# adithom/KWS

Measured on AMD Instinct MI355X. Metric: utterances/sec fwd+bwd, T=99 feat=32 hidden=128, bs=4096 at 1/2/4/8 GPUs, higher is better.
Workload: dtype f32 (split-precision MFMA: exact 3xbf16 planes, fp16 two-plane forward state product; fp32 accumulate)

## Files before the change

include/fastgrnn_hip.h:

```cpp
#ifndef FASTGRNN_HIP_H
#define FASTGRNN_HIP_H

#include <stddef.h>
#include <stdint.h>

#ifdef __cplusplus
extern "C" {
#endif

#define FASTGRNN_HIP_ABI_VERSION 1

typedef enum fastgrnn_status {
  FASTGRNN_OK = 0,
  FASTGRNN_ERR_NULL_POINTER = 1,
  FASTGRNN_ERR_BAD_SHAPE = 2,
  FASTGRNN_ERR_BAD_NONLINEARITY = 3,
  FASTGRNN_ERR_BAD_DTYPE = 4,
  FASTGRNN_ERR_WORKSPACE = 5,
  FASTGRNN_ERR_LAUNCH = 6,
  FASTGRNN_ERR_UNSUPPORTED = 7
} fastgrnn_status;

typedef enum fastgrnn_dtype {
  FASTGRNN_F32 = 0,
  FASTGRNN_F64 = 1,
  FASTGRNN_BF16_IO = 2
} fastgrnn_dtype;

typedef enum fastgrnn_nonlinearity {
  FASTGRNN_NL_SIGMOID = 0, FASTGRNN_NL_RELU = 1, FASTGRNN_NL_TANH = 2,
  FASTGRNN_NL_QUANT_TANH = 3, FASTGRNN_NL_QUANT_SIGM = 4, FASTGRNN_NL_QUANT_SIGM4 = 5
} fastgrnn_nonlinearity;

#define FASTGRNN_FLAG_FORCE_GENERIC 1u
#define FASTGRNN_FLAG_FORCE_F32_MFMA 2u
#define FASTGRNN_FLAG_SAVE_PREACT 4u
#define FASTGRNN_FLAG_FWD_4WAVE 8u
#define FASTGRNN_FLAG_BATCH_MAJOR 16u
#define FASTGRNN_FLAG_X_BFT 128u
#define FASTGRNN_FLAG_FWD_BF16X3 64u
#define FASTGRNN_FLAG_GRAD_LAST 256u
#define FASTGRNN_FLAG_HS_LAST 512u
#define FASTGRNN_FLAG_PREACT_AFFINE 1024u
#define FASTGRNN_FLAG_BN_TRAIN 2048u
#define FASTGRNN_FLAG_ZERO_EXTEND 4096u
#define FASTGRNN_FLAG_NO_INPUT_GRAD 8192u

typedef struct fastgrnn_desc {
  int32_t T, B, F, H;
  int32_t w_rank, u_rank;
  int32_t gate_nl;
  int32_t update_nl;
  int32_t dtype;
  uint32_t flags;
} fastgrnn_desc;

typedef struct fastgrnn_params {
  const void *w, *u;
  const void *w1, *w2, *u1, *u2;
  const void *bias_gate;
  const void *bias_update;
  const void *zeta, *nu;
} fastgrnn_params;

typedef struct fastgrnn_grads {
  void *d_x;
  void *d_bias_gate;
  void *d_bias_update;
  void *d_zeta;
  void *d_nu;
  void *d_h0;
  void *d_w, *d_u;
  void *d_w1, *d_w2;
  void *d_u1, *d_u2;
} fastgrnn_grads;

int fastgrnn_hip_abi_version(void);
const char *fastgrnn_hip_status_string(int status);

int fastgrnn_hip_kernel_path(const fastgrnn_desc *d, int direction);

typedef struct fastgrnn_zext_plan {
  int32_t forward, backward;
  int32_t Hp, Fp;
  int32_t dx_optional, reserved;
  size_t saved_bytes;
} fastgrnn_zext_plan;
int fastgrnn_hip_zero_extend_plan(const fastgrnn_desc *d, fastgrnn_zext_plan *out);

typedef struct fastgrnn_plan {
// ... 224 lines not shown
```

kws_amd/_lib.py:

```python
from __future__ import annotations

import ctypes as C
import os

_HERE = os.path.dirname(os.path.abspath(__file__))
LIB_PATH = os.environ.get("FASTGRNN_HIP_LIB") or os.path.join(_HERE, "csrc", "libfastgrnn_hip.so")

ABI_VERSION = 1

F32, F64, BF16_IO = 0, 1, 2
FLAG_FORCE_GENERIC = 1
FLAG_FORCE_F32_MFMA = 2
FLAG_SAVE_PREACT = 4
FLAG_FWD_4WAVE = 8
FLAG_FWD_BF16X3 = 64
FLAG_X_BFT = 128
FLAG_GRAD_LAST = 256
FLAG_HS_LAST = 512
FLAG_BATCH_MAJOR = 16
FLAG_PREACT_AFFINE = 1024
FLAG_BN_TRAIN = 2048
FLAG_ZERO_EXTEND = 4096
FLAG_NO_INPUT_GRAD = 8192

NONLINEARITY = {"sigmoid": 0, "relu": 1, "tanh": 2, "quantTanh": 3, "quantSigm": 4, "quantSigm4": 5}

EXPORTS = (
    "fastgrnn_hip_abi_version", "fastgrnn_hip_status_string", "fastgrnn_hip_kernel_path",
    "fastgrnn_hip_forward_workspace_bytes", "fastgrnn_hip_backward_workspace_bytes",
    "fastgrnn_hip_forward_unroll", "fastgrnn_hip_backward_unroll",
    "fastgrnn_hip_forward", "fastgrnn_hip_backward",
    "fastgrnn_hip_head_workspace_bytes", "fastgrnn_hip_head_xent", "fastgrnn_hip_debug_poison_cu_state",
    "fastgrnn_hip_frame_gemm", "fastgrnn_hip_forward_unroll_affine",
    "fastgrnn_hip_bn_train_supported", "fastgrnn_hip_bn_train_forward_workspace_bytes",
    "fastgrnn_hip_bn_train_backward_workspace_bytes", "fastgrnn_hip_bn_train_forward", "fastgrnn_hip_bn_train_backward",
    "fastgrnn_hip_zero_extend_plan", "fastgrnn_hip_plan",
    "fastgrnn_hip_windows_supported", "fastgrnn_hip_forward_windows_workspace_bytes", "fastgrnn_hip_forward_windows",
    "fastgrnn_hip_train_windows_supported", "fastgrnn_hip_train_windows_forward_workspace_bytes",
    "fastgrnn_hip_train_windows_backward_workspace_bytes", "fastgrnn_hip_forward_windows_train",
    "fastgrnn_hip_backward_windows",
    "fastgrnn_hip_head_predict_workspace_bytes", "fastgrnn_hip_head_predict", "fastgrnn_hip_vote_windows",
    "fastgrnn_hip_train_update", "fastgrnn_hip_optim_update",
    "fastgrnn_hip_mfcc_tables_bytes", "fastgrnn_hip_mfcc_init_tables", "fastgrnn_hip_mfcc_workspace_bytes",
    "fastgrnn_hip_mfcc", "fastgrnn_hip_mfcc_augment", "fastgrnn_hip_augment_draw", "fastgrnn_hip_train_schedule",
)


class Desc(C.Structure):
    _fields_ = [("T", C.c_int32), ("B", C.c_int32), ("F", C.c_int32), ("H", C.c_int32),
                ("w_rank", C.c_int32), ("u_rank", C.c_int32),
                ("gate_nl", C.c_int32), ("update_nl", C.c_int32),
                ("dtype", C.c_int32), ("flags", C.c_uint32)]


class Params(C.Structure):
    _fields_ = [(n, C.c_void_p) for n in
                ("w", "u", "w1", "w2", "u1", "u2", "bias_gate", "bias_update", "zeta", "nu")]


class Grads(C.Structure):
    _fields_ = [(n, C.c_void_p) for n in
                ("d_x", "d_bias_gate", "d_bias_update", "d_zeta", "d_nu", "d_h0",
                 "d_w", "d_u", "d_w1", "d_w2", "d_u1", "d_u2")]


class BnLayer(C.Structure):
    _fields_ = [("gamma", C.c_void_p), ("beta", C.c_void_p), ("running_mean", C.c_void_p),
                ("running_var", C.c_void_p), ("num_batches_tracked", C.c_void_p),
                ("eps", C.c_double), ("momentum", C.c_double)]


class BnParams(C.Structure):
    _fields_ = [("w", BnLayer), ("u", BnLayer), ("gate", BnLayer), ("update", BnLayer)]


class BnGrads(C.Structure):
# ... 208 lines not shown
```

kws_amd/csrc/kernels_split.hip:

```cpp
#include "split_common.h"

namespace fastgrnn {
namespace {

template <int GATE, int AUX, bool RAGGED>
__global__ __launch_bounds__(256) ONE_WAVE_PER_SIMD void fwd_scan_split(
    int Tn, int B, int rsT, int rsB, const float* __restrict__ x, const float* __restrict__ h0,
    const float* __restrict__ w, const float* __restrict__ u,
    const float* __restrict__ bz, const float* __restrict__ bh,
    const float* __restrict__ zeta, const float* __restrict__ nu,
    float* __restrict__ hs, float* __restrict__ zs, float* __restrict__ cs) {
  constexpr int H = 128, F = 32, MT = 2, KS = H / 32;
  __shared__ u32x4 hl[2][3][KS * 4 * 16];

  const int tid = threadIdx.x;
  const int wv = __builtin_amdgcn_readfirstlane(tid >> 6);
  const int l = tid & 63, i = l & 15, g = l >> 4;
  const int b = blockIdx.x * 16 + i;
  const bool valid = !RAGGED || b < B;
  const int bc = valid ? b : B - 1;
  const int n0 = wv * 32 + g * 8;
  const int myfrag = (wv * 4 + g) * 16 + i;

  Frag3 Uf[MT][KS], Wf[MT];
// ... 364 lines not shown
      st4(zs + o, zq); st4(cs + o, cq);
    }
    aux_prev = a;
    publish_h(cur ^ 1);
    SPLIT_STAMP(3)
    lds_barrier();
    SPLIT_STAMP(4)
  }
#ifdef FASTGRNN_DIAG_STAMPS
  if (blockIdx.x == 7 && l == 0) { for (int k2 = 0; k2 < 8; ++k2) g_sdiag[wv][k2] = dsum[k2]; }
#endif
  store_step(Tn - 1, aux_prev);
  };
  if constexpr (F16H) {
    if (use_h16) scan(std::true_type{}); else scan(std::false_type{});
  } else {
    scan(std::false_type{});
  }
}



constexpr int SLAB = (128 * 128 + 128 * 32 + 2 * 128 + 2 + 63) & ~63;

constexpr int ROW_H = 288;
constexpr int ROW_X = 96;
constexpr int PLANE_H = 16 * ROW_H;
constexpr int PLANE_X = 16 * ROW_X;
constexpr int IMG = 2 * 3 * PLANE_H + 3 * PLANE_X;

constexpr int OFF_DP = 0, OFF_HP = 3 * PLANE_H, OFF_XP = 6 * PLANE_H;

template <bool WITH_DX>
struct BwdW8Lds {
  unsigned char img[4][IMG];
  f32x4 DX[2][8][64];
  float bias[2][128];
  float red[16];
};
template <>
struct BwdW8Lds<false> {
  unsigned char img[4][IMG];
  float bias[2][128];
  float red[16];
};

constexpr bool bwd_w8_built(int gate, bool preact, bool bf, bool nox, bool uq, bool nodx) {
  const bool ref_gate = gate <= FASTGRNN_NL_TANH;
  if (nox) return !uq && !nodx && (!bf || (ref_gate && preact));
  if (uq) return preact && !bf;
  if (bf) return preact;
  return true;
}
template <int GATE, bool PREACT, bool RAGGED, bool BF = false, bool NOX = false, bool UQ = false, bool NODX = false>
__global__ __launch_bounds__(512) void bwd_scan_split_w8(
    int Tn, int B, int rsT, int rsB, int mode, const float* __restrict__ ghs, const float* __restrict__ x,
    const float* __restrict__ hs, const float* __restrict__ aux0, const float* __restrict__ aux1,
    const float* __restrict__ h0, const float* __restrict__ w, const float* __restrict__ u,
    const float* __restrict__ bz, const float* __restrict__ bh,
    const float* __restrict__ zeta, const float* __restrict__ nu,
    float* __restrict__ d_x, float* __restrict__ d_h0, float* __restrict__ part) {
  constexpr int H = 128, F = 32, KS = 4, NFT = NOX ? 0 : 2, NC = NOX ? 4 : 5;
  constexpr bool STATIC_TURNS = !NOX, SELECT_AT_USE = !NOX;
  static_assert(!(NOX && NODX), "NOX scans leave d_x to a GEMM of its own");
  __shared__ BwdW8Lds<!NODX> S;
#ifdef FASTGRNN_DIAG_STAMPS
  unsigned long long dsum[8] = {0, 0, 0, 0, 0, 0, 0, 0}, dlast = 0;
  asm volatile("s_memtime %0\n\ts_waitcnt lgkmcnt(0)" : "=s"(dlast)::"memory");
#endif

  const bool xbft = (mode & 1) != 0, g_last = (mode & 2) != 0;
  const int tid = threadIdx.x;
  const int wv = __builtin_amdgcn_readfirstlane(tid >> 6);
  const int l = tid & 63, i = l & 15, g = l >> 4;
  const int b = blockIdx.x * 16 + i;
  const bool valid = !RAGGED || b < B;
  const int bc = valid ? b : B - 1;
  const int n0 = wv * 16 + g * 4;
  const float sz = fsigmoid(zeta[0]), sn = fsigmoid(nu[0]);
  if (Tn & 1) {
    for (int idx = tid; idx < IMG / 4; idx += 512) reinterpret_cast<unsigned*>(&S.img[Tn & 3][0])[idx] = 0u;
  }
  if (PREACT && tid < 256) S.bias[tid >> 7][tid & 127] = (tid < 128 ? bz : bh)[tid & 127];

  Frag3 UTf[KS];
#pragma unroll
  for (int s2 = 0; s2 < KS; ++s2) {
    f32x4 lo, hi;
#pragma unroll
    for (int j = 0; j < 4; ++j) {
      lo[j] = u[(size_t)(32 * s2 + 8 * g + j) * H + wv * 16 + i];
      hi[j] = u[(size_t)(32 * s2 + 8 * g + 4 + j) * H + wv * 16 + i];
    }
    UTf[s2] = split3(lo, hi);
  }
  const int xf2 = wv & 1, xks = wv >> 1;
  Frag3 WTf;
  if (!NOX && !NODX) {
    f32x4 lo, hi;
#pragma unroll
    for (int j = 0; j < 4; ++j) {
      lo[j] = w[(size_t)(32 * xks + 8 * g + j) * F + xf2 * 16 + i];
      hi[j] = w[(size_t)(32 * xks + 8 * g + 4 + j) * F + xf2 * 16 + i];
    }
    WTf = split3(lo, hi);
  }
  f32x4 sbz = f32x4{0.f, 0.f, 0.f, 0.f}, sbh = sbz, dh = sbz;
  float pz = 0.f, pn = 0.f, pz_c = 0.f, pn_c = 0.f;
  auto role_body = [&](auto role_tag) __attribute__((always_inline)) {
  const int rp = wv & 3;
  constexpr int ch = decltype(role_tag)::value;
  f32x4 acc[2][NC];
#pragma unroll
  for (int a = 0; a < 2; ++a)
#pragma unroll
    for (int c = 0; c < NC; ++c) acc[a][c] = f32x4{0.f, 0.f, 0.f, 0.f};

  const unsigned lds_img = (unsigned)(size_t)&S.img[0][0];
  const unsigned my_row_h = (unsigned)(i * ROW_H + n0 * 2);
  const int xu = tid >> 5, xf = tid & 31;
  const unsigned my_x = (unsigned)(xu * ROW_X + xf * 2);
  const int xbb = blockIdx.x * 16 + xu;
  const int xbc = (!RAGGED || xbb < B) ? xbb : B - 1;
  const int q = (l & 15) >> 2, pp = l & 3;
  const unsigned trA_off = OFF_DP + (8 * (g & 1) + q) * ROW_H + (rp * 32 + 4 * pp) * 2;
  const unsigned trH_off = OFF_HP + (8 * (g & 1) + q) * ROW_H + (4 * pp) * 2;
  const unsigned trX_off = OFF_XP + (8 * (g & 1) + q) * ROW_X + (4 * pp) * 2;

  auto fragments_landed = [&]() __attribute__((always_inline)) { __builtin_amdgcn_sched_barrier(0); };
  struct EwOps { f32x4 g, a0, a1, h; float xv; uint2 graw, hraw; unsigned short xraw; };
  constexpr unsigned ESZ = BF ? 2u : 4u;
  const unsigned lane_e = (unsigned)bc * (unsigned)rsB * H + n0;
  const unsigned lane_bh = (unsigned)bc * H + n0;
  const unsigned dp_step = (NOX && valid) ? (unsigned)rsT * H * 4u : 0u;
  const unsigned dp_off = !NOX ? 0u : (valid ? ((unsigned)b * (unsigned)rsB * H + n0) * 4u
                                             : (((unsigned)Tn * (unsigned)B + i) * H + n0) * 4u);
  const unsigned lane_x = NOX ? 0u : (xbft ? ((unsigned)xbc * F + xf) * (unsigned)Tn : (unsigned)xbc * (unsigned)rsB * F + xf);
  auto ldg4 = [](const void* base, unsigned byte_off) __attribute__((always_inline)) {
    return *reinterpret_cast<const f32x4*>(reinterpret_cast<const char*>(base) + byte_off);
  };
  auto ldg2 = [](const void* base, unsigned byte_off) __attribute__((always_inline)) {
    return *reinterpret_cast<const uint2*>(reinterpret_cast<const char*>(base) + byte_off);
  };
  auto load_ew = [&](int t, EwOps& e) __attribute__((always_inline)) {
    const size_t step_h = (size_t)t * rsT * H;
    e.a0 = ldg4(aux0 + step_h, lane_e * 4u);
    if (!PREACT) e.a1 = ldg4(aux1 + step_h, lane_e * 4u);
    const char* gbase = g_last ? reinterpret_cast<const char*>(ghs) : reinterpret_cast<const char*>(ghs) + step_h * ESZ;
    const unsigned goff = (g_last ? lane_bh : lane_e) * ESZ;
    const char* hbase = (t == 0) ? reinterpret_cast<const char*>(hs)
                                 : reinterpret_cast<const char*>(hs) + (step_h - (size_t)rsT * H) * ESZ;
    const char* xbase = xbft ? reinterpret_cast<const char*>(x) + (size_t)t * ESZ
                             : reinterpret_cast<const char*>(x) + (size_t)t * rsT * F * ESZ;
    const bool g_zero = g_last && t != Tn - 1;
    if (BF) {
      e.graw = ldg2(gbase, goff);
      if constexpr (!SELECT_AT_USE) {
        e.graw = g_zero ? uint2{0u, 0u} : e.graw;
        if (RAGGED && !valid) e.graw = uint2{0u, 0u};
      }
      e.hraw = ldg2(hbase, lane_e * ESZ);
      if (t == 0) e.h = ldg4(h0, lane_bh * 4u);
      if (!NOX) e.xraw = *reinterpret_cast<const unsigned short*>(xbase + lane_x * ESZ);
    } else {
      e.g = ldg4(gbase, goff);
      if constexpr (!SELECT_AT_USE) {
        e.g = g_zero ? f32x4{0.f, 0.f, 0.f, 0.f} : e.g;
        if (RAGGED && !valid) e.g = f32x4{0.f, 0.f, 0.f, 0.f};
      }
      e.h = (t == 0) ? ldg4(h0, lane_bh * 4u) : ldg4(hbase, lane_e * 4u);
      if (!NOX) e.xv = *reinterpret_cast<const float*>(xbase + lane_x * 4u);
    }
  };
  auto unpack4 = [](const uint2 v) __attribute__((always_inline)) {
    return f32x4{__builtin_bit_cast(float, v.x << 16), __builtin_bit_cast(float, v.x & 0xFFFF0000u),
                 __builtin_bit_cast(float, v.y << 16), __builtin_bit_cast(float, v.y & 0xFFFF0000u)};
  };
  auto unpack_ew = [&](int t, EwOps& e) __attribute__((always_inline)) {
    if (BF) {
      e.g = unpack4(e.graw);
      if (t != 0) e.h = unpack4(e.hraw);
      if (!NOX) e.xv = bf16_to_f32(e.xraw);
    }
    if constexpr (SELECT_AT_USE) {
      const bool g_zero = g_last && t != Tn - 1;
      e.g = g_zero ? f32x4{0.f, 0.f, 0.f, 0.f} : e.g;
      if (RAGGED && !valid) e.g = f32x4{0.f, 0.f, 0.f, 0.f};
    }
  };
  struct EwPre { f32x4 kc, kz, z, c; };
  auto ew_pre = [&](const EwOps& e, EwPre& f) __attribute__((always_inline)) {
    f32x4 bzq = f32x4{0.f, 0.f, 0.f, 0.f}, bhq = bzq;
    if (PREACT) {
      bzq = *reinterpret_cast<const f32x4*>(&S.bias[0][n0]);
      bhq = *reinterpret_cast<const f32x4*>(&S.bias[1][n0]);
    }
#pragma unroll
    for (int r = 0; r < 4; ++r) {
      float z, c;
      if (PREACT) {
        z = gate_act<GATE>(e.a0[r] + bzq[r]);
        c = UQ ? fminf(fmaxf(e.a0[r] + bhq[r], -1.0f), 1.0f) : ftanh(e.a0[r] + bhq[r]);
      } else {
        z = e.a0[r]; c = e.a1[r];
      }
      const float dc = UQ ? ((c < 1.0f && c > -1.0f) ? 1.0f : 0.0f) : 1.0f - c * c;
      f.kc[r] = (sz * (1.0f - z) + sn) * dc;
      f.kz[r] = (e.h[r] - sz * c) * gate_dact<GATE>(z);
      f.z[r] = z; f.c[r] = c;
    }
  };
  auto put4 = [&](unsigned char* base, int plane_stride, unsigned off, const f32x4 v) __attribute__((always_inline)) {
    uint2 q0, q1, q2;
    split_quad(v, q0, q1, q2);
    *reinterpret_cast<uint2*>(base + off) = q0;
    *reinterpret_cast<uint2*>(base + plane_stride + off) = q1;
    *reinterpret_cast<uint2*>(base + 2 * plane_stride + off) = q2;
  };
  auto ew_post = [&](int t, const EwOps& e, const EwPre& f, const f32x4 ggv) __attribute__((always_inline)) {
    f32x4 dpv;
    float sn4 = 0.f, sz4 = 0.f;
#pragma unroll
    for (int r = 0; r < 4; ++r) {
      const float gg = ggv[r];
      const float dcp = f.kc[r] * gg, dzp = f.kz[r] * gg;
      sbz[r] += dzp; sbh[r] += dcp;
      const float cg = f.c[r] * gg;
      if constexpr (NOX) { sn4 += cg; sz4 += cg - f.z[r] * cg; }
      else { pn += cg; pz += cg - f.z[r] * cg; }
      dpv[r] = dzp + dcp;
      dh[r] = f.z[r] * gg;
    }
    if constexpr (NOX) { kahan_add(pn, pn_c, sn4); kahan_add(pz, pz_c, sz4); }
    unsigned char* im = &S.img[t & 3][0];
    put4(im + OFF_DP, PLANE_H, my_row_h, dpv);
    put4(im + OFF_HP, PLANE_H, my_row_h, e.h);
    if (NOX) {
      *reinterpret_cast<f32x4*>(reinterpret_cast<char*>(d_x) + (size_t)t * dp_step + dp_off) = dpv;
    } else {
      unsigned short s0, s1, s2;
      split_one(e.xv, s0, s1, s2);
      *reinterpret_cast<unsigned short*>(im + OFF_XP + my_x) = s0;
      *reinterpret_cast<unsigned short*>(im + OFF_XP + PLANE_X + my_x) = s1;
      *reinterpret_cast<unsigned short*>(im + OFF_XP + 2 * PLANE_X + my_x) = s2;
    }
  };
  auto finish_dx = [&](int t) __attribute__((always_inline)) {
    if constexpr (!NOX && !NODX) {
      if (wv < NFT) {
        const f32x4 sacc = (S.DX[t & 1][wv][l] + S.DX[t & 1][wv + 2][l]) + (S.DX[t & 1][wv + 4][l] + S.DX[t & 1][wv + 6][l]);
        if (xbft) {
          if (valid) {
#pragma unroll
            for (int r = 0; r < 4; ++r) {
              const size_t o = ((size_t)b * F + wv * 16 + 4 * g + r) * Tn + t;
              if (BF) reinterpret_cast<unsigned short*>(d_x)[o] = (unsigned short)f32_to_bf16_rne(sacc[r]);
              else d_x[o] = sacc[r];
            }
          }
        } else {
          char* xo = reinterpret_cast<char*>(d_x) + (size_t)t * rsT * F * ESZ;
          const unsigned lo = ((unsigned)b * (unsigned)rsB * F + wv * 16 + 4 * g) * ESZ;
          if (valid) { if (BF) st4_bf16(xo + lo, sacc); else *reinterpret_cast<f32x4*>(xo + lo) = sacc; }
        }
      }
    }
  };
  auto weight_grads = [&](auto pure_tag, int sU) __attribute__((always_inline)) {
    constexpr bool PURE3 = decltype(pure_tag)::value;
    const unsigned im = lds_img + (unsigned)(((g < 2) ? sU : sU - 1) & 3) * IMG;
    const unsigned trA = im + trA_off, trH = im + trH_off, trX = im + trX_off;
    Frag3 Af[2];
#pragma unroll
    for (int a2 = 0; a2 < 2; ++a2)
#pragma unroll
      for (int pl = 0; pl < 3; ++pl) Af[a2].p[pl] = tr_frag(trA + pl * PLANE_H + a2 * 32, ROW_H);
    auto load_b = [&](int c, Frag3& bf) __attribute__((always_inline)) {
      const int ct = NC * ch + c;
#pragma unroll
      for (int pl = 0; pl < 3; ++pl)
        bf.p[pl] = (ct < NFT) ? tr_frag(trX + pl * PLANE_X + ct * 32, ROW_X)
                              : tr_frag(trH + pl * PLANE_H + (ct - NFT) * 32, ROW_H);
    };
    auto batch = [&](auto c0_tag, auto n_tag) __attribute__((always_inline)) {
      constexpr int C0 = decltype(c0_tag)::value, NB = decltype(n_tag)::value;
      Frag3 Bf[NB];
#pragma unroll
      for (int c = 0; c < NB; ++c) load_b(C0 + c, Bf[c]);
      fragments_landed();
      if constexpr (PURE3) {
#pragma unroll
        for (int c = 0; c < NB; ++c)
#pragma unroll
          for (int a2 = 0; a2 < 2; ++a2) {
            f32x4 v = mfma_bf16(Af[a2].p[2], Bf[c].p[0], acc[a2][C0 + c]);
            v = mfma_bf16(Af[a2].p[1], Bf[c].p[0], v);
            acc[a2][C0 + c] = mfma_bf16(Af[a2].p[0], Bf[c].p[0], v);
          }
      } else {
#pragma unroll
        for (int c = 0; c < NB; ++c)
#pragma unroll
          for (int a2 = 0; a2 < 2; ++a2) acc[a2][C0 + c] = mfma6(Af[a2], Bf[c], acc[a2][C0 + c]);
      }
      __builtin_amdgcn_sched_barrier(0);
      float touch = 0.f;
#pragma unroll
      for (int c = 0; c < NB; ++c) touch += acc[0][C0 + c][0] + acc[1][C0 + c][0];
      completion_read(touch);
      __builtin_amdgcn_sched_barrier(0);
    };
    constexpr bool ONE_TILE_BATCHES = PREACT && GATE == FASTGRNN_NL_TANH && !NOX;
    if constexpr (ONE_TILE_BATCHES) {
      static_for<NC>([&](auto c_tag) __attribute__((always_inline)) { batch(c_tag, std::integral_constant<int, 1>{}); });
    } else {
      batch(std::integral_constant<int, 0>{}, std::integral_constant<int, 2>{});
      batch(std::integral_constant<int, 2>{}, std::integral_constant<int, 2>{});
      if constexpr (NC == 5) batch(std::integral_constant<int, 4>{}, std::integral_constant<int, 1>{});
    }
  };

  const int top = (Tn & 1) ? Tn : Tn - 1;
  auto iter = [&](auto last_tag, auto even_tag, auto peeled_tag, int t, EwOps& eo) __attribute__((always_inline)) {
    constexpr bool LAST = decltype(last_tag)::value, EVEN = decltype(even_tag)::value, PEELED = decltype(peeled_tag)::value;
    SPLIT_STAMP(0)
    constexpr bool MY_TURN = EVEN ? (ch == 0) : (ch == 1);
    constexpr bool HEAVY = MY_TURN && !PEELED;
    const unsigned char* im = &S.img[t & 3][0];
    Frag3 dB[KS];
#pragma unroll
    for (int s2 = 0; s2 < KS; ++s2)
#pragma unroll
      for (int p = 0; p < 3; ++p)
        dB[s2].p[p] = *reinterpret_cast<const u32x4*>(im + OFF_DP + p * PLANE_H + i * ROW_H + (32 * s2 + 8 * g) * 2);
    if (t + 1 < Tn) finish_dx(t + 1);
    fragments_landed();
    SPLIT_STAMP(1)
    EwPre f;
    auto chain = [&]() __attribute__((always_inline)) {
      const f32x4 z4 = f32x4{0.f, 0.f, 0.f, 0.f};
      f32x4 dlo = z4;
#pragma unroll
      for (int s2 = 0; s2 < KS; ++s2) mfma6_hl(UTf[s2], dB[s2], dh, dlo);
      dh += dlo;
      asm volatile("" : "+v"(dh));
      if constexpr (!NOX && !NODX) {
        f32x4 dxp;
        static_assert(KS == 4, "four K-steps");
        if (xks == 0) dxp = mfma6(WTf, dB[0], z4);
        else if (xks == 1) dxp = mfma6(WTf, dB[1], z4);
        else if (xks == 2) dxp = mfma6(WTf, dB[2], z4);
        else dxp = mfma6(WTf, dB[3], z4);
        S.DX[t & 1][wv][l] = dxp;
      }
    };
    chain();
    __builtin_amdgcn_sched_barrier(0);
    if constexpr (!LAST) { unpack_ew(t - 1, eo); ew_pre(eo, f); }
    __builtin_amdgcn_sched_barrier(0);
    SPLIT_STAMP(2)
    if constexpr (!LAST) {
      ew_post(t - 1, eo, f, eo.g + dh);
      __builtin_amdgcn_sched_barrier(0);
      if (BF) lds_writes_landed();
      load_ew(t >= 2 ? t - 2 : 0, eo);
    }
    __builtin_amdgcn_sched_barrier(0);
    SPLIT_STAMP(3)
    if constexpr (STATIC_TURNS) {
      if constexpr (HEAVY) weight_grads(std::bool_constant<BF && !LAST>{}, EVEN ? t + 1 : t + 2);
    } else {
      if (MY_TURN && (EVEN || t + 2 <= top)) weight_grads(std::bool_constant<BF && !LAST>{}, EVEN ? t + 1 : t + 2);
    }
    SPLIT_STAMP(4)
    lds_barrier();
    SPLIT_STAMP(5)
  };

  EwOps E;
  __syncthreads();
  {
    EwPre f;
    load_ew(Tn - 1, E);
    unpack_ew(Tn - 1, E); ew_pre(E, f); ew_post(Tn - 1, E, f, E.g);
    __builtin_amdgcn_sched_barrier(0);
    if (Tn >= 2) load_ew(Tn - 2, E);
  }
  __syncthreads();
  {
    int t = Tn - 1;
    if (t & 1) { iter(std::false_type{}, std::false_type{}, std::true_type{}, t, E); --t; }
    for (; t >= 2; t -= 2) {
      iter(std::false_type{}, std::true_type{}, std::false_type{}, t, E);
      iter(std::false_type{}, std::false_type{}, std::false_type{}, t - 1, E);
    }
    iter(std::true_type{}, std::true_type{}, std::false_type{}, 0, E);
  }
#ifdef FASTGRNN_DIAG_STAMPS
  if (blockIdx.x == 7 && l == 0) { for (int k2 = 0; k2 < 8; ++k2) g_sdiag[wv][k2] = dsum[k2]; }
#endif
  if constexpr (ch == 1) weight_grads(std::false_type{}, 1);
  finish_dx(0);
  if (valid) st4(d_h0 + (size_t)b * H + n0, dh);
  {
    float* pu = part + (size_t)blockIdx.x * SLAB;
    float* pw = pu + H * H;
#pragma unroll
    for (int a = 0; a < 2; ++a)
#pragma unroll
      for (int r = 0; r < 4; ++r) {
        const int n = rp * 32 + a * 16 + 4 * g + r;
#pragma unroll
        for (int c = 0; c < NC; ++c) {
          const int ct = NC * ch + c;
          if (ct < NFT) pw[(size_t)n * F + ct * 16 + i] = acc[a][c][r];
          else pu[(size_t)n * H + (ct - NFT) * 16 + i] = acc[a][c][r];
        }
      }
  }
  };
  if (wv < 4) role_body(std::integral_constant<int, 0>{}); else role_body(std::integral_constant<int, 1>{});
#pragma unroll
  for (int r = 0; r < 4; ++r) {
    float a = sbz[r], c = sbh[r];
#pragma unroll
    for (int m = 1; m < 16; m <<= 1) { a += __shfl_xor(a, m); c += __shfl_xor(c, m); }
    if (i == 0) {
      float* pb = part + (size_t)blockIdx.x * SLAB + H * H + H * F;
      pb[n0 + r] = a;
      pb[H + n0 + r] = c;
    }
  }
#pragma unroll
  for (int m = 1; m < 64; m <<= 1) { pz += __shfl_xor(pz, m); pn += __shfl_xor(pn, m); }
  if (l == 0) { S.red[wv] = pz; S.red[8 + wv] = pn; }
  __syncthreads();
  if (tid == 0) {
    float* pzn = part + (size_t)blockIdx.x * SLAB + H * H + H * F + 2 * H;
    float a = 0.f, c = 0.f;
#pragma unroll
    for (int k = 0; k < 8; ++k) { a += S.red[k]; c += S.red[8 + k]; }
    pzn[0] = a; pzn[1] = c;
  }
}

__global__ __launch_bounds__(1024) void reduce_slabs_split(int nwg, const float* __restrict__ part,
                                                           const float* __restrict__ zeta, const float* __restrict__ nu,
                                                           float* __restrict__ d_u, float* __restrict__ d_w,
                                                           float* __restrict__ d_bz, float* __restrict__ d_bh,
                                                           float* __restrict__ d_zeta, float* __restrict__ d_nu) {
  constexpr int H = 128, F = 32;
  __shared__ float sm[16][64];
  const int o = threadIdx.x & 63, part_id = threadIdx.x >> 6;
  const int idx = blockIdx.x * 64 + o;
  const int ntot = H * H + H * F + 2 * H + 2;
  float a = 0.f;
  if (idx < ntot) {
    float v[8];
    for (int wg0 = part_id; wg0 < nwg; wg0 += 16 * 8) {
#pragma unroll
      for (int j = 0; j < 8; ++j) {
        const int wg = wg0 + 16 * j;
        v[j] = wg < nwg ? part[(size_t)wg * SLAB + idx] : 0.f;
      }
      a += ((v[0] + v[1]) + (v[2] + v[3])) + ((v[4] + v[5]) + (v[6] + v[7]));
    }
  }
  sm[part_id][o] = a;
  __syncthreads();
  if (part_id == 0 && idx < ntot) {
    float t = 0.f;
#pragma unroll
    for (int j = 0; j < 16; ++j) t += sm[j][o];
    const int oW = H * H, oBz = oW + H * F, oBh = oBz + H, oZ = oBh + H;
    if (idx < oW) d_u[idx] = t;
    else if (idx < oBz) { if (d_w) d_w[idx - oW] = t; }
    else if (idx < oBh) d_bz[idx - oBz] = t;
    else if (idx < oZ) d_bh[idx - oBh] = t;
    else if (idx == oZ) { const float sz = 1.0f / (1.0f + expf(-zeta[0])); d_zeta[0] = t * sz * (1.0f - sz); }
    else { const float sn = 1.0f / (1.0f + expf(-nu[0])); d_nu[0] = t * sn * (1.0f - sn); }
  }
}

bool dense_wide_shape(const fastgrnn_desc& d) {
  return d.w_rank == 0 && d.u_rank == 0 && d.H == 128 && (d.F == 64 || d.F == 128 || d.F == 256) &&
         ((double)d.T * d.B + 16.0) * (d.F > 128 ? d.F : 128) * 4.0 < 4294967296.0;
}
bool dense_f32_shape(const fastgrnn_desc& d) { return d.w_rank == 0 && d.u_rank == 0 && d.H == 128 && d.F == 32 && seq_fits32(d); }

DpreBwdWs w8_bwd_ws(const fastgrnn_desc& d, void* base) {
  if (dense_wide_shape(d)) return dpre_bwd_ws(d, SLAB, false, base);
  Carve c(base);
  DpreBwdWs L{};
  L.part = c.take<float>((size_t)((d.B + 15) / 16) * SLAB);
  L.bytes = c.off;
  return L;
}
struct WideFwdWs { float* P; size_t bytes; };
WideFwdWs wide_fwd_ws(const fastgrnn_desc& d, void* base) {
  Carve c(base);
  float* P = c.take<float>((size_t)d.T * d.B * 128);
  return {P, c.off};
}
struct GatherWs { char* inner; float* xg; size_t bytes; };
GatherWs gather_ws(const fastgrnn_desc& d, size_t inner_bytes, void* base) {
  Carve c(base);
  char* inner = c.take<char>(inner_bytes);
  float* xg = c.take<float>((size_t)d.T * d.B * d.F);
  return {inner, xg, c.off};
}

struct BwdW8 { int gate; bool preact, ragged, bf, nox, uq, nodx; };

int launch_bwd_w8(const fastgrnn_desc& d, const fastgrnn_params& p, const void* ghs, const void* x, const void* hs,
                  const void* a0, const void* a1, const void* h0, const fastgrnn_grads& g, void* ws, hipStream_t s) {
  const int nwg = (d.B + 15) / 16;
  dim3 grid(nwg);
  const bool wide = dense_wide_shape(d);
  const DpreBwdWs L = w8_bwd_ws(d, ws);
  float* const part = L.part, * const dpre = L.dpre;
  auto go8 = [&](auto kern) __attribute__((always_inline)) {
    hipLaunchKernelGGL(kern, grid, dim3(512), 0, s, d.T, d.B, row_stride_t(d), row_stride_b(d),
                       ((d.flags & FASTGRNN_FLAG_X_BFT) ? 1 : 0) | ((d.flags & FASTGRNN_FLAG_GRAD_LAST) ? 2 : 0), (const float*)ghs,
                       (const float*)x, (const float*)hs,
                       (const float*)a0, (const float*)a1, (const float*)h0, (const float*)p.w, (const float*)p.u,
                       (const float*)p.bias_gate, (const float*)p.bias_update, (const float*)p.zeta,
                       (const float*)p.nu, wide ? dpre : (float*)g.d_x, (float*)g.d_h0, part);
  };
  const BwdW8 v{d.gate_nl, (d.flags & FASTGRNN_FLAG_SAVE_PREACT) != 0, (d.B % 16) != 0, d.dtype == FASTGRNN_BF16_IO,
                wide, d.update_nl == FASTGRNN_NL_QUANT_TANH, !wide && g.d_x == nullptr};
  const bool launched =
      pick_int<0, 1, 2, 3, 4, 5>(v.gate, [&](auto G_) {
      return pick_bool(v.preact, [&](auto PA_) {
      return pick_bool(v.bf, [&](auto BF_) {
      return pick_bool(v.nox, [&](auto NX_) {
      return pick_bool(v.uq, [&](auto UQ_) {
      return pick_bool(v.nodx, [&](auto ND_) {
      return pick_bool(v.ragged, [&](auto RG_) {
        constexpr int G = decltype(G_)::value;
        constexpr bool PA = decltype(PA_)::value, BF = decltype(BF_)::value, NX = decltype(NX_)::value,
                       UQ = decltype(UQ_)::value, ND = decltype(ND_)::value, RG = decltype(RG_)::value;
        if constexpr (bwd_w8_built(G, PA, BF, NX, UQ, ND)) { go8(bwd_scan_split_w8<G, PA, RG, BF, NX, UQ, ND>); return true; }
        else return false;
      }); }); }); }); }); }); });
  if (!launched) return FASTGRNN_ERR_UNSUPPORTED;
  const int ntot = 128 * 128 + 128 * 32 + 2 * 128 + 2;
  hipLaunchKernelGGL(reduce_slabs_split, dim3((ntot + 63) / 64), dim3(1024), 0, s, nwg, part, (const float*)p.zeta,
                     (const float*)p.nu, (float*)g.d_u, wide ? (float*)nullptr : (float*)g.d_w, (float*)g.d_bias_gate,
                     (float*)g.d_bias_update, (float*)g.d_zeta, (float*)g.d_nu);
  if (wide) {
    const int st = dpre_bwd_tail(d, dpre, L.tn, L.xtm, x, p.w, g, s);
    if (st) return st;
  }
  return launch_status();
}

struct FwdW8 { int gate, aux; bool ragged, bf, f16h, prein, uq, aff, win; };

int launch_fwd(const fastgrnn_desc& d, const fastgrnn_params& p, const void* x, const void* h0, void* hs,
               void* zs, void* cs, hipStream_t s, void* pws, const float* sg, const float* sc,
               const window_src* win = nullptr) {
  dim3 grid((d.B + 15) / 16), block(256);
  const bool ragged = (d.B % 16) != 0, bf = d.dtype == FASTGRNN_BF16_IO, prein = pws != nullptr;
  const int aux = zs == nullptr ? 0 : ((d.flags & FASTGRNN_FLAG_SAVE_PREACT) ? 2 : 1);
  if (prein && aux == 0) zs = pws;
  auto go = [&](auto kern) __attribute__((always_inline)) {
    hipLaunchKernelGGL(kern, grid, block, 0, s, d.T, d.B, row_stride_t(d), row_stride_b(d), (const float*)x,
                       (const float*)h0, (const float*)p.w,
                       (const float*)p.u, (const float*)p.bias_gate, (const float*)p.bias_update,
                       (const float*)p.zeta, (const float*)p.nu, (float*)hs, (float*)zs, (float*)cs);
  };
  auto go8 = [&](auto kern) __attribute__((always_inline)) {
    hipLaunchKernelGGL(kern, grid, dim3(512), 0, s, d.T, d.B, row_stride_t(d), row_stride_b(d),
                       (d.flags & FASTGRNN_FLAG_X_BFT) ? 1 : 0, (const float*)x, (const float*)h0, (const float*)p.w,
                       (const float*)p.u, (const float*)p.bias_gate, (const float*)p.bias_update,
                       (const float*)p.zeta, (const float*)p.nu, (float*)hs, (float*)zs, (float*)cs, sg, sc,
                       win ? win->start : nullptr);
  };
  if ((d.flags & FASTGRNN_FLAG_FWD_4WAVE) && !win && !sg && !bf && d.gate_nl <= FASTGRNN_NL_TANH &&
      !(d.flags & (FASTGRNN_FLAG_X_BFT | FASTGRNN_FLAG_HS_LAST | FASTGRNN_FLAG_FWD_BF16X3)))
    return pick_int<0, 1, 2>(d.gate_nl, [&](auto G_) {
           return pick_int<0, 1, 2>(aux, [&](auto A_) {
           return pick_bool(ragged, [&](auto RG_) {
             go(fwd_scan_split<decltype(G_)::value, decltype(A_)::value, decltype(RG_)::value>);
             return true;
           }); }); }) ? launch_status() : FASTGRNN_ERR_UNSUPPORTED;
  const FwdW8 v{d.gate_nl, (d.flags & FASTGRNN_FLAG_HS_LAST) ? 3 : aux, ragged, bf,
                gate_bounds_state(d.gate_nl) && !(d.flags & FASTGRNN_FLAG_FWD_BF16X3), prein,
                d.update_nl == FASTGRNN_NL_QUANT_TANH, sg != nullptr, win != nullptr};
  const bool launched =
         pick_int<0, 1, 2, 3, 4, 5>(v.gate, [&](auto G_) {
         return pick_int<0, 1, 2, 3>(v.aux, [&](auto A_) {
         return pick_bool(v.bf, [&](auto BF_) {
         return pick_bool(v.f16h, [&](auto FH_) {
         return pick_bool(v.prein, [&](auto PI_) {
         return pick_bool(v.uq, [&](auto UQ_) {
         return pick_bool(v.aff, [&](auto AF_) {
// ... 167 lines not shown
```

Measured before the change: 11.60 million.

## Offload backward weight-gradient MFMAs to four helper waves in a 12-wave scan

Adds a 768-thread variant of the backward scan for the no-input-gradient F=32 case. Four extra helper waves do all weight-gradient MFMA accumulation from the shared LDS images, and the eight recurrence waves only run the serial time scan at raised scheduling priority. The aim is to take the weight-gradient work off the critical recurrence path. In exchange it uses more threads and registers per workgroup, which may lower occupancy. A flag keeps the old 8-wave kernel available.

```diff
diff --git a/include/fastgrnn_hip.h b/include/fastgrnn_hip.h
--- a/include/fastgrnn_hip.h
+++ b/include/fastgrnn_hip.h
@@ -36,6 +36,7 @@
 #define FASTGRNN_FLAG_FORCE_F32_MFMA 2u
 #define FASTGRNN_FLAG_SAVE_PREACT 4u
 #define FASTGRNN_FLAG_FWD_4WAVE 8u
+#define FASTGRNN_FLAG_BWD_8WAVE 32u
 #define FASTGRNN_FLAG_BATCH_MAJOR 16u
 #define FASTGRNN_FLAG_X_BFT 128u
 #define FASTGRNN_FLAG_FWD_BF16X3 64u
diff --git a/kws_amd/_lib.py b/kws_amd/_lib.py
--- a/kws_amd/_lib.py
+++ b/kws_amd/_lib.py
@@ -22,6 +22,7 @@
 FLAG_BN_TRAIN = 2048
 FLAG_ZERO_EXTEND = 4096
 FLAG_NO_INPUT_GRAD = 8192
+AB_BWD_8WAVE = 32
 
 NONLINEARITY = {"sigmoid": 0, "relu": 1, "tanh": 2, "quantTanh": 3, "quantSigm": 4, "quantSigm4": 5}
 
diff --git a/kws_amd/csrc/kernels_split.hip b/kws_amd/csrc/kernels_split.hip
--- a/kws_amd/csrc/kernels_split.hip
+++ b/kws_amd/csrc/kernels_split.hip
@@ -440,8 +440,9 @@
   if (bf) return preact;
   return true;
 }
-template <int GATE, bool PREACT, bool RAGGED, bool BF = false, bool NOX = false, bool UQ = false, bool NODX = false>
-__global__ __launch_bounds__(512) void bwd_scan_split_w8(
+constexpr int W12_RECURRENCE_PRIO = 1;
+template <int GATE, bool PREACT, bool RAGGED, bool BF, bool NOX, bool UQ, bool NODX, bool HW>
+__device__ __forceinline__ void bwd_scan_split_body(
     int Tn, int B, int rsT, int rsB, int mode, const float* __restrict__ ghs, const float* __restrict__ x,
     const float* __restrict__ hs, const float* __restrict__ aux0, const float* __restrict__ aux1,
     const float* __restrict__ h0, const float* __restrict__ w, const float* __restrict__ u,
@@ -449,6 +450,8 @@
     const float* __restrict__ zeta, const float* __restrict__ nu,
     float* __restrict__ d_x, float* __restrict__ d_h0, float* __restrict__ part) {
   constexpr int H = 128, F = 32, KS = 4, NFT = NOX ? 0 : 2, NC = NOX ? 4 : 5;
+  constexpr int NT = HW ? 768 : 512;
+  static_assert(!HW || (NODX && !NOX), "helper waves: the F = 32 scans without d_x");
   constexpr bool STATIC_TURNS = !NOX, SELECT_AT_USE = !NOX;
   static_assert(!(NOX && NODX), "NOX scans leave d_x to a GEMM of its own");
   __shared__ BwdW8Lds<!NODX> S;
@@ -467,20 +470,23 @@
   const int n0 = wv * 16 + g * 4;
   const float sz = fsigmoid(zeta[0]), sn = fsigmoid(nu[0]);
   if (Tn & 1) {
-    for (int idx = tid; idx < IMG / 4; idx += 512) reinterpret_cast<unsigned*>(&S.img[Tn & 3][0])[idx] = 0u;
-  }
+    for (int idx = tid; idx < IMG / 4; idx += NT) reinterpret_cast<unsigned*>(&S.img[Tn & 3][0])[idx] = 0u;
+  }
+  const bool helper = HW && wv >= 8;
   if (PREACT && tid < 256) S.bias[tid >> 7][tid & 127] = (tid < 128 ? bz : bh)[tid & 127];
 
   Frag3 UTf[KS];
-#pragma unroll
-  for (int s2 = 0; s2 < KS; ++s2) {
-    f32x4 lo, hi;
-#pragma unroll
-    for (int j = 0; j < 4; ++j) {
-      lo[j] = u[(size_t)(32 * s2 + 8 * g + j) * H + wv * 16 + i];
-      hi[j] = u[(size_t)(32 * s2 + 8 * g + 4 + j) * H + wv * 16 + i];
-    }
-    UTf[s2] = split3(lo, hi);
+  if (!helper) {
+#pragma unroll
+    for (int s2 = 0; s2 < KS; ++s2) {
+      f32x4 lo, hi;
+#pragma unroll
+      for (int j = 0; j < 4; ++j) {
+        lo[j] = u[(size_t)(32 * s2 + 8 * g + j) * H + wv * 16 + i];
+        hi[j] = u[(size_t)(32 * s2 + 8 * g + 4 + j) * H + wv * 16 + i];
+      }
+      UTf[s2] = split3(lo, hi);
+    }
   }
   const int xf2 = wv & 1, xks = wv >> 1;
   Frag3 WTf;
@@ -495,14 +501,24 @@
   }
   f32x4 sbz = f32x4{0.f, 0.f, 0.f, 0.f}, sbh = sbz, dh = sbz;
   float pz = 0.f, pn = 0.f, pz_c = 0.f, pn_c = 0.f;
+  struct LaneId { int i, n0, b; bool valid; };
+  auto lane_again = [&]() __attribute__((always_inline)) {
+    int t2 = tid;
+    if constexpr (HW) asm volatile("" : "+v"(t2));
+    const int i2 = t2 & 15, b2 = blockIdx.x * 16 + i2;
+    return LaneId{i2, __builtin_amdgcn_readfirstlane(t2 >> 6) * 16 + ((t2 & 63) >> 4) * 4, b2, !RAGGED || b2 < B};
+  };
   auto role_body = [&](auto role_tag) __attribute__((always_inline)) {
   const int rp = wv & 3;
-  constexpr int ch = decltype(role_tag)::value;
-  f32x4 acc[2][NC];
+  constexpr int role = decltype(role_tag)::value;
+  constexpr bool HELPER = role == 3, WG = role != 2;
+  constexpr int ch = role & 1;
+  constexpr int NA = HELPER ? 2 * NC : NC;
+  f32x4 acc[2][NA];
 #pragma unroll
   for (int a = 0; a < 2; ++a)
 #pragma unroll
-    for (int c = 0; c < NC; ++c) acc[a][c] = f32x4{0.f, 0.f, 0.f, 0.f};
+    for (int c = 0; c < NA; ++c) acc[a][c] = f32x4{0.f, 0.f, 0.f, 0.f};
 
   const unsigned lds_img = (unsigned)(size_t)&S.img[0][0];
   const unsigned my_row_h = (unsigned)(i * ROW_H + n0 * 2);
@@ -524,11 +540,15 @@
   const unsigned dp_off = !NOX ? 0u : (valid ? ((unsigned)b * (unsigned)rsB * H + n0) * 4u
                                              : (((unsigned)Tn * (unsigned)B + i) * H + n0) * 4u);
   const unsigned lane_x = NOX ? 0u : (xbft ? ((unsigned)xbc * F + xf) * (unsigned)Tn : (unsigned)xbc * (unsigned)rsB * F + xf);
-  auto ldg4 = [](const void* base, unsigned byte_off) __attribute__((always_inline)) {
-    return *reinterpret_cast<const f32x4*>(reinterpret_cast<const char*>(base) + byte_off);
-  };
-  auto ldg2 = [](const void* base, unsigned byte_off) __attribute__((always_inline)) {
-    return *reinterpret_cast<const uint2*>(reinterpret_cast<const char*>(base) + byte_off);
+  auto off32 = [](unsigned byte_off) __attribute__((always_inline)) {
+    if constexpr (HW) asm volatile("" : "+v"(byte_off));
+    return byte_off;
+  };
+  auto ldg4 = [&](const void* base, unsigned byte_off) __attribute__((always_inline)) {
+    return *reinterpret_cast<const f32x4*>(reinterpret_cast<const char*>(base) + off32(byte_off));
+  };
+  auto ldg2 = [&](const void* base, unsigned byte_off) __attribute__((always_inline)) {
+    return *reinterpret_cast<const uint2*>(reinterpret_cast<const char*>(base) + off32(byte_off));
   };
   auto load_ew = [&](int t, EwOps& e) __attribute__((always_inline)) {
     const size_t step_h = (size_t)t * rsT * H;
@@ -549,15 +569,16 @@
       }
       e.hraw = ldg2(hbase, lane_e * ESZ);
       if (t == 0) e.h = ldg4(h0, lane_bh * 4u);
-      if (!NOX) e.xraw = *reinterpret_cast<const unsigned short*>(xbase + lane_x * ESZ);
+      if (!NOX) e.xraw = *reinterpret_cast<const unsigned short*>(xbase + off32(lane_x * ESZ));
     } else {
       e.g = ldg4(gbase, goff);
       if constexpr (!SELECT_AT_USE) {
         e.g = g_zero ? f32x4{0.f, 0.f, 0.f, 0.f} : e.g;
         if (RAGGED && !valid) e.g = f32x4{0.f, 0.f, 0.f, 0.f};
       }
-      e.h = (t == 0) ? ldg4(h0, lane_bh * 4u) : ldg4(hbase, lane_e * 4u);
-      if (!NOX) e.xv = *reinterpret_cast<const float*>(xbase + lane_x * 4u);
+      if constexpr (HW) e.h = ldg4((t == 0) ? reinterpret_cast<const char*>(h0) : hbase, ((t == 0) ? lane_bh : lane_e) * 4u);
+      else e.h = (t == 0) ? ldg4(h0, lane_bh * 4u) : ldg4(hbase, lane_e * 4u);
+      if (!NOX) e.xv = *reinterpret_cast<const float*>(xbase + off32(lane_x * 4u));
     }
   };
   auto unpack4 = [](const uint2 v) __attribute__((always_inline)) {
@@ -654,8 +675,9 @@
       }
     }
   };
-  auto weight_grads = [&](auto pure_tag, int sU) __attribute__((always_inline)) {
+  auto weight_grads = [&](auto pure_tag, auto half_tag, int sU) __attribute__((always_inline)) {
     constexpr bool PURE3 = decltype(pure_tag)::value;
+    constexpr int CH = decltype(half_tag)::value, A0 = HELPER ? NC * CH : 0;
     const unsigned im = lds_img + (unsigned)(((g < 2) ? sU : sU - 1) & 3) * IMG;
     const unsigned trA = im + trA_off, trH = im + trH_off, trX = im + trX_off;
     Frag3 Af[2];
@@ -664,7 +686,7 @@
 #pragma unroll
       for (int pl = 0; pl < 3; ++pl) Af[a2].p[pl] = tr_frag(trA + pl * PLANE_H + a2 * 32, ROW_H);
     auto load_b = [&](int c, Frag3& bf) __attribute__((always_inline)) {
-      const int ct = NC * ch + c;
+      const int ct = NC * CH + c;
 #pragma unroll
       for (int pl = 0; pl < 3; ++pl)
         bf.p[pl] = (ct < NFT) ? tr_frag(trX + pl * PLANE_X + ct * 32, ROW_X)
@@ -681,20 +703,20 @@
         for (int c = 0; c < NB; ++c)
 #pragma unroll
           for (int a2 = 0; a2 < 2; ++a2) {
-            f32x4 v = mfma_bf16(Af[a2].p[2], Bf[c].p[0], acc[a2][C0 + c]);
+            f32x4 v = mfma_bf16(Af[a2].p[2], Bf[c].p[0], acc[a2][A0 + C0 + c]);
             v = mfma_bf16(Af[a2].p[1], Bf[c].p[0], v);
-            acc[a2][C0 + c] = mfma_bf16(Af[a2].p[0], Bf[c].p[0], v);
+            acc[a2][A0 + C0 + c] = mfma_bf16(Af[a2].p[0], Bf[c].p[0], v);
           }
       } else {
 #pragma unroll
         for (int c = 0; c < NB; ++c)
 #pragma unroll
-          for (int a2 = 0; a2 < 2; ++a2) acc[a2][C0 + c] = mfma6(Af[a2], Bf[c], acc[a2][C0 + c]);
+          for (int a2 = 0; a2 < 2; ++a2) acc[a2][A0 + C0 + c] = mfma6(Af[a2], Bf[c], acc[a2][A0 + C0 + c]);
       }
       __builtin_amdgcn_sched_barrier(0);
       float touch = 0.f;
 #pragma unroll
-      for (int c = 0; c < NB; ++c) touch += acc[0][C0 + c][0] + acc[1][C0 + c][0];
+      for (int c = 0; c < NB; ++c) touch += acc[0][A0 + C0 + c][0] + acc[1][A0 + C0 + c][0];
       completion_read(touch);
       __builtin_amdgcn_sched_barrier(0);
     };
@@ -713,7 +735,7 @@
     constexpr bool LAST = decltype(last_tag)::value, EVEN = decltype(even_tag)::value, PEELED = decltype(peeled_tag)::value;
     SPLIT_STAMP(0)
     constexpr bool MY_TURN = EVEN ? (ch == 0) : (ch == 1);
-    constexpr bool HEAVY = MY_TURN && !PEELED;
+    constexpr bool HEAVY = WG && MY_TURN && !PEELED;
     const unsigned char* im = &S.img[t & 3][0];
     Frag3 dB[KS];
 #pragma unroll
@@ -756,15 +778,32 @@
     __builtin_amdgcn_sched_barrier(0);
     SPLIT_STAMP(3)
     if constexpr (STATIC_TURNS) {
-      if constexpr (HEAVY) weight_grads(std::bool_constant<BF && !LAST>{}, EVEN ? t + 1 : t + 2);
+      if constexpr (HEAVY) weight_grads(std::bool_constant<BF && !LAST>{}, role_tag, EVEN ? t + 1 : t + 2);
     } else {
-      if (MY_TURN && (EVEN || t + 2 <= top)) weight_grads(std::bool_constant<BF && !LAST>{}, EVEN ? t + 1 : t + 2);
+      if (MY_TURN && (EVEN || t + 2 <= top)) weight_grads(std::bool_constant<BF && !LAST>{}, role_tag, EVEN ? t + 1 : t + 2);
     }
     SPLIT_STAMP(4)
     lds_barrier();
     SPLIT_STAMP(5)
   };
 
+  if constexpr (HELPER) {
+    __syncthreads();
+    __syncthreads();
+    constexpr std::integral_constant<int, 0> h0_tag{};
+    constexpr std::integral_constant<int, 1> h1_tag{};
+    int t = Tn - 1;
+    if (t & 1) { lds_barrier(); --t; }
+    for (; t >= 2; t -= 2) {
+      weight_grads(std::bool_constant<BF>{}, h0_tag, t + 1);
+      lds_barrier();
+      weight_grads(std::bool_constant<BF>{}, h1_tag, t + 1);
+      lds_barrier();
+    }
+    weight_grads(std::false_type{}, h0_tag, 1);
+    lds_barrier();
+    weight_grads(std::false_type{}, h1_tag, 1);
+  } else {
   EwOps E;
   __syncthreads();
   {
@@ -775,6 +814,7 @@
     if (Tn >= 2) load_ew(Tn - 2, E);
   }
   __syncthreads();
+  if constexpr (HW && W12_RECURRENCE_PRIO > 0) __builtin_amdgcn_s_setprio(W12_RECURRENCE_PRIO);
   {
     int t = Tn - 1;
     if (t & 1) { iter(std::false_type{}, std::false_type{}, std::true_type{}, t, E); --t; }
@@ -787,10 +827,14 @@
 #ifdef FASTGRNN_DIAG_STAMPS
   if (blockIdx.x == 7 && l == 0) { for (int k2 = 0; k2 < 8; ++k2) g_sdiag[wv][k2] = dsum[k2]; }
 #endif
-  if constexpr (ch == 1) weight_grads(std::false_type{}, 1);
+  if constexpr (WG && ch == 1) weight_grads(std::false_type{}, role_tag, 1);
   finish_dx(0);
-  if (valid) st4(d_h0 + (size_t)b * H + n0, dh);
   {
+    const LaneId q = lane_again();
+    if (q.valid) st4(d_h0 + (size_t)q.b * H + q.n0, dh);
+  }
+  }
+  if constexpr (WG) {
     float* pu = part + (size_t)blockIdx.x * SLAB;
     float* pw = pu + H * H;
 #pragma unroll
@@ -799,29 +843,36 @@
       for (int r = 0; r < 4; ++r) {
         const int n = rp * 32 + a * 16 + 4 * g + r;
 #pragma unroll
-        for (int c = 0; c < NC; ++c) {
-          const int ct = NC * ch + c;
+        for (int c = 0; c < NA; ++c) {
+          const int ct = HELPER ? c : NC * ch + c;
           if (ct < NFT) pw[(size_t)n * F + ct * 16 + i] = acc[a][c][r];
           else pu[(size_t)n * H + (ct - NFT) * 16 + i] = acc[a][c][r];
         }
       }
   }
   };
-  if (wv < 4) role_body(std::integral_constant<int, 0>{}); else role_body(std::integral_constant<int, 1>{});
-#pragma unroll
-  for (int r = 0; r < 4; ++r) {
-    float a = sbz[r], c = sbh[r];
-#pragma unroll
-    for (int m = 1; m < 16; m <<= 1) { a += __shfl_xor(a, m); c += __shfl_xor(c, m); }
-    if (i == 0) {
-      float* pb = part + (size_t)blockIdx.x * SLAB + H * H + H * F;
-      pb[n0 + r] = a;
-      pb[H + n0 + r] = c;
-    }
-  }
-#pragma unroll
-  for (int m = 1; m < 64; m <<= 1) { pz += __shfl_xor(pz, m); pn += __shfl_xor(pn, m); }
-  if (l == 0) { S.red[wv] = pz; S.red[8 + wv] = pn; }
+  if constexpr (HW) {
+    if (helper) role_body(std::integral_constant<int, 3>{}); else role_body(std::integral_constant<int, 2>{});
+  } else {
+    if (wv < 4) role_body(std::integral_constant<int, 0>{}); else role_body(std::integral_constant<int, 1>{});
+  }
+  if (!helper) {
+    const LaneId q = lane_again();
+#pragma unroll
+    for (int r = 0; r < 4; ++r) {
+      float a = sbz[r], c = sbh[r];
+#pragma unroll
+      for (int m = 1; m < 16; m <<= 1) { a += __shfl_xor(a, m); c += __shfl_xor(c, m); }
+      if (q.i == 0) {
+        float* pb = part + (size_t)blockIdx.x * SLAB + H * H + H * F;
+        pb[q.n0 + r] = a;
+        pb[H + q.n0 + r] = c;
+      }
+    }
+#pragma unroll
+    for (int m = 1; m < 64; m <<= 1) { pz += __shfl_xor(pz, m); pn += __shfl_xor(pn, m); }
+    if (l == 0) { S.red[wv] = pz; S.red[8 + wv] = pn; }
+  }
   __syncthreads();
   if (tid == 0) {
     float* pzn = part + (size_t)blockIdx.x * SLAB + H * H + H * F + 2 * H;
@@ -831,6 +882,29 @@
     pzn[0] = a; pzn[1] = c;
   }
 }
+
+#define BWD_SCAN_ARGS                                                                                             \
+  int Tn, int B, int rsT, int rsB, int mode, const float* __restrict__ ghs, const float* __restrict__ x,           \
+      const float* __restrict__ hs, const float* __restrict__ aux0, const float* __restrict__ aux1,                \
+      const float* __restrict__ h0, const float* __restrict__ w, const float* __restrict__ u,                      \
+      const float* __restrict__ bz, const float* __restrict__ bh, const float* __restrict__ zeta,                  \
+      const float* __restrict__ nu, float* __restrict__ d_x, float* __restrict__ d_h0, float* __restrict__ part
+#define BWD_SCAN_PASS Tn, B, rsT, rsB, mode, ghs, x, hs, aux0, aux1, h0, w, u, bz, bh, zeta, nu, d_x, d_h0, part
+
+template <int GATE, bool PREACT, bool RAGGED, bool BF = false, bool NOX = false, bool UQ = false, bool NODX = false>
+__global__ __launch_bounds__(512) void bwd_scan_split_w8(BWD_SCAN_ARGS) {
+  bwd_scan_split_body<GATE, PREACT, RAGGED, BF, NOX, UQ, NODX, false>(BWD_SCAN_PASS);
+}
+
+constexpr bool bwd_w12_built(int gate, bool preact, bool bf, bool nox, bool uq, bool nodx) {
+  return nodx && !nox && !bf && !uq && gate <= FASTGRNN_NL_TANH && bwd_w8_built(gate, preact, bf, nox, uq, nodx);
+}
+template <int GATE, bool PREACT, bool RAGGED, bool BF = false, bool UQ = false>
+__global__ __launch_bounds__(768) void bwd_scan_split_w12(BWD_SCAN_ARGS) {
+  bwd_scan_split_body<GATE, PREACT, RAGGED, BF, false, UQ, true, true>(BWD_SCAN_PASS);
+}
+#undef BWD_SCAN_ARGS
+#undef BWD_SCAN_PASS
 
 __global__ __launch_bounds__(1024) void reduce_slabs_split(int nwg, const float* __restrict__ part,
                                                            const float* __restrict__ zeta, const float* __restrict__ nu,
@@ -898,7 +972,7 @@
   return {inner, xg, c.off};
 }
 
-struct BwdW8 { int gate; bool preact, ragged, bf, nox, uq, nodx; };
+struct BwdW8 { int gate; bool preact, ragged, bf, nox, uq, nodx, w12; };
 
 int launch_bwd_w8(const fastgrnn_desc& d, const fastgrnn_params& p, const void* ghs, const void* x, const void* hs,
                   const void* a0, const void* a1, const void* h0, const fastgrnn_grads& g, void* ws, hipStream_t s) {
@@ -907,16 +981,17 @@
   const bool wide = dense_wide_shape(d);
   const DpreBwdWs L = w8_bwd_ws(d, ws);
   float* const part = L.part, * const dpre = L.dpre;
-  auto go8 = [&](auto kern) __attribute__((always_inline)) {
-    hipLaunchKernelGGL(kern, grid, dim3(512), 0, s, d.T, d.B, row_stride_t(d), row_stride_b(d),
+  auto go8 = [&](auto kern, int waves) __attribute__((always_inline)) {
+    hipLaunchKernelGGL(kern, grid, dim3(64 * waves), 0, s, d.T, d.B, row_stride_t(d), row_stride_b(d),
                        ((d.flags & FASTGRNN_FLAG_X_BFT) ? 1 : 0) | ((d.flags & FASTGRNN_FLAG_GRAD_LAST) ? 2 : 0), (const float*)ghs,
                        (const float*)x, (const float*)hs,
                        (const float*)a0, (const float*)a1, (const float*)h0, (const float*)p.w, (const float*)p.u,
                        (const float*)p.bias_gate, (const float*)p.bias_update, (const float*)p.zeta,
                        (const float*)p.nu, wide ? dpre : (float*)g.d_x, (float*)g.d_h0, part);
   };
-  const BwdW8 v{d.gate_nl, (d.flags & FASTGRNN_FLAG_SAVE_PREACT) != 0, (d.B % 16) != 0, d.dtype == FASTGRNN_BF16_IO,
-                wide, d.update_nl == FASTGRNN_NL_QUANT_TANH, !wide && g.d_x == nullptr};
+  BwdW8 v{d.gate_nl, (d.flags & FASTGRNN_FLAG_SAVE_PREACT) != 0, (d.B % 16) != 0, d.dtype == FASTGRNN_BF16_IO,
+          wide, d.update_nl == FASTGRNN_NL_QUANT_TANH, !wide && g.d_x == nullptr, false};
+  v.w12 = !(d.flags & FASTGRNN_FLAG_BWD_8WAVE) && bwd_w12_built(v.gate, v.preact, v.bf, v.nox, v.uq, v.nodx);
   const bool launched =
       pick_int<0, 1, 2, 3, 4, 5>(v.gate, [&](auto G_) {
       return pick_bool(v.preact, [&](auto PA_) {
@@ -924,13 +999,18 @@
       return pick_bool(v.nox, [&](auto NX_) {
       return pick_bool(v.uq, [&](auto UQ_) {
       return pick_bool(v.nodx, [&](auto ND_) {
+      return pick_bool(v.w12, [&](auto W12_) {
       return pick_bool(v.ragged, [&](auto RG_) {
         constexpr int G = decltype(G_)::value;
         constexpr bool PA = decltype(PA_)::value, BF = decltype(BF_)::value, NX = decltype(NX_)::value,
-                       UQ = decltype(UQ_)::value, ND = decltype(ND_)::value, RG = decltype(RG_)::value;
-        if constexpr (bwd_w8_built(G, PA, BF, NX, UQ, ND)) { go8(bwd_scan_split_w8<G, PA, RG, BF, NX, UQ, ND>); return true; }
+                       UQ = decltype(UQ_)::value, ND = decltype(ND_)::value, W12 = decltype(W12_)::value,
+                       RG = decltype(RG_)::value;
+        if constexpr (W12) {
+          if constexpr (bwd_w12_built(G, PA, BF, NX, UQ, ND)) { go8(bwd_scan_split_w12<G, PA, RG, BF, UQ>, 12); return true; }
+          else return false;
+        } else if constexpr (bwd_w8_built(G, PA, BF, NX, UQ, ND)) { go8(bwd_scan_split_w8<G, PA, RG, BF, NX, UQ, ND>, 8); return true; }
         else return false;
-      }); }); }); }); }); }); });
+      }); }); }); }); }); }); }); });
   if (!launched) return FASTGRNN_ERR_UNSUPPORTED;
   const int ntot = 128 * 128 + 128 * 32 + 2 * 128 + 2;
   hipLaunchKernelGGL(reduce_slabs_split, dim3((ntot + 63) / 64), dim3(1024), 0, s, nwg, part, (const float*)p.zeta,
```

After: 12.13 million (median of 6 runs). +4.5%, better.
